# heracles-ec/heracles

Measured on AMD Instinct MI355X. Metric: map->Cl pairs/sec + mixing-matrix build sec, nside=4096 lmax=6144, higher is better.
Workload: dtype f64

## Files before the change

### heracles_amd/csrc/hx_analysis.hip

```cpp
#include <algorithm>
#include <cmath>
#include <cstdlib>
#include <cstring>

#include "hx_sht_common.h"

namespace hx {
using namespace hxfft;

constexpr int HALF_F = 1;
template <int SPIN>
struct LegCfg {
    static constexpr int NW = SPIN == 0 ? 16 : 8;
    static constexpr int NT = SPIN == 0 ? 1 : 2;
    static constexpr int NOP = SPIN == 0 ? 1 : 2;
    static constexpr int NPAR = (SPIN == 2 && HALF_F) ? 1 : 2;
};
int analysis_f_rows(int spin) { return spin == 0 ? LegCfg<0>::NPAR * LegCfg<0>::NOP : LegCfg<2>::NPAR * LegCfg<2>::NOP; }

struct LegParams {
    PlanDev P;
    const LegTask *__restrict__ tasks;
    const double *__restrict__ F;
    double *__restrict__ partial;
    int m0, ms;
    long long row0;
    int ng;
    int ncol;
    int pcol;
    const MTasks *__restrict__ of_m;
    const long long *__restrict__ arow;
    long long arow0;
    int add_all;
};

template <int SPIN>
__global__ __launch_bounds__(256) void k_fourier_combine(PlanDev P, const double2 *__restrict__ Y, int ncomp, int ng,
                                                         int ncol, int m0, int ms, const double *__restrict__ rw,
                                                         const LegTask *__restrict__ tasks, const MTasks *__restrict__ of_m,
                                                         double *__restrict__ F, int tile0)
{
    constexpr int NOP = LegCfg<SPIN>::NOP;
    __shared__ RingAtM ring_at_m[32];
    const int m = m0 + blockIdx.x * ms;
    const int ty = (int)blockIdx.y + tile0;
    const MTasks mt = of_m[m];
    if (mt.count == 0 || ty < tasks[mt.first].rb0) return;
    if (threadIdx.x < 32) ring_at_m[threadIdx.x] = ring_at_m_of(P, ty * 32 + threadIdx.x, m, rw);
    __syncthreads();
    const int rp = ty * 32 + (threadIdx.x >> 3);
    const int slot = threadIdx.x & 7;
    const bool live = rp < P.nrp;
    const RingAtM ram = ring_at_m[threadIdx.x >> 3];
    constexpr int NPAR = LegCfg<SPIN>::NPAR;
    double *row = F + (((long long)blockIdx.x * P.nrp_pad + rp) * NPAR) * NOP * ncol;
    for (int g = 0; g < ng; ++g) {
        if (SPIN == 0) {
            const int c = g * 8 + slot;
            if (g * NCOL + 2 * slot >= ncol) continue;
            double2 s = make_double2(0.0, 0.0), d = s;
            if (live && c < ncomp) {
                double2 fn, fs;
                ring_modes_ns(P, Y, c, rp, m, ram, fn, fs);
                s = cadd(fn, fs);
                d = csub(fn, fs);
            }
            *reinterpret_cast<double2 *>(row + g * NCOL + 2 * slot) = s;
            *reinterpret_cast<double2 *>(row + ncol + g * NCOL + 2 * slot) = d;
        } else {
            const int f = g * 4 + (slot >> 1), op = slot & 1;
            if (g * NCOL + 4 * (slot >> 1) >= ncol) continue;
            double4 o0 = make_double4(0.0, 0.0, 0.0, 0.0), o1 = o0;
            if (live && 2 * f + 1 < ncomp) {
                double2 qn, qs, un, us;
                ring_modes_ns(P, Y, 2 * f, rp, m, ram, qn, qs);
                ring_modes_ns(P, Y, 2 * f + 1, rp, m, ram, un, us);
                const double2 ppn = cscale(cadd(qn, mul_pi(un)), -0.5), pmn = cscale(csub(qn, mul_pi(un)), -0.5);
                const double2 pps = cscale(cadd(qs, mul_pi(us)), -0.5), pms = cscale(csub(qs, mul_pi(us)), -0.5);
                double4 x, y;
                if (op == 0) {
                    x = make_double4(ppn.x, ppn.y, ppn.y, -ppn.x);
                    y = make_double4(pms.x, pms.y, -pms.y, pms.x);
                } else {
                    x = make_double4(pmn.x, pmn.y, -pmn.y, pmn.x);
                    y = make_double4(pps.x, pps.y, pps.y, -pps.x);
                }
                o0 = make_double4(x.x + y.x, x.y + y.y, x.z + y.z, x.w + y.w);
                o1 = make_double4(x.x - y.x, x.y - y.y, x.z - y.z, x.w - y.w);
            }
            const int col = g * NCOL + 4 * (slot >> 1);
            *reinterpret_cast<double4 *>(row + (0 * NOP + op) * ncol + col) = o0;
            if (NPAR == 2) *reinterpret_cast<double4 *>(row + (1 * NOP + op) * ncol + col) = o1;
        }
    }
}

__device__ __host__ inline int tile_swz(int r) { return r & 15; }
__device__ __host__ inline int ringsel(int q, int k) { return (k & 1) * 16 + 2 * q + (k >> 1); }

template <int K>
__device__ inline int opaque(int v)
{
    asm("; opaque %1" : "+v"(v) : "n"(K));
    return v;
}

__device__ unsigned long long g_exec_flops[2];

template <int SPIN>
struct PipeCfg {
    static constexpr int NW = 4;
    static constexpr int RBS = SPIN == 0 ? 2 : 1;
    static constexpr int NCH = SPIN == 0 ? 2 : 1;
    static constexpr int NOP = SPIN == 0 ? 1 : 2;
};

__device__ __host__ inline int pipe_rho(int q, int k) { return 4 * q + k; }
__device__ __host__ inline int pipe_tile_idx(int c, int r) { return c * 32 + ((r ^ (c & 7)) * 2); }

constexpr int DUO_GAP = -1;
constexpr int DUO_PRIO = 1;
constexpr int DUO_ORDER = -1;
constexpr int DUO_SCALE_BITS2 = 100;
constexpr int DUO_SCALE_BITS0 = 300;

template <int K>
__device__ __forceinline__ double row_bcast(double v)
{
    double d;
    asm("v_mov_b64_dpp %0, %1 row_newbcast:%2 row_mask:0xf bank_mask:0xf" : "=v"(d) : "v"(v), "n"(K));
    return d;
}

template <int K>
__device__ __forceinline__ double row_bcast_fmac(double t, double p, double x)
{
    asm("v_fmac_f64_dpp %0, %1, %2 row_newbcast:%3 row_mask:0xf bank_mask:0xf" : "+v"(t) : "v"(p), "v"(x), "n"(K));
    return t;
}

template <int SPIN>
__device__ __forceinline__ void alm_rows_to_layout(const PlanDev &P, int m, bool any_task, const double *__restrict__ partial, long long r0, int ncol,
                                                   int ncomp, int ng, const double *__restrict__ fl, int add, double2 *__restrict__ alm,
                                                   long long alm_stride, const double *__restrict__ alphan, int tid, int nt)
{
    const int lmax = P.lmax;
    const int l0 = SPIN == 0 ? m : (m > 2 ? m : 2);
    const int nl = lmax - m + 1, nc = 8 * ng;
    constexpr int U = 8;
    for (int i0 = tid; i0 < nl * nc; i0 += nt * U) {
        double2 v[U];
        double al[U], f[U];
        long long dsti[U];
        bool on[U];
#pragma unroll
        for (int u = 0; u < U; ++u) {
            const int i = i0 + u * nt;
            const int l = m + i / nc, c = i % nc;
            on[u] = i < nl * nc && c < ncomp;
            v[u] = make_double2(0.0, 0.0);
            al[u] = 1.0;
            f[u] = 1.0;
            dsti[u] = 0;
            if (!on[u]) continue;
            dsti[u] = (long long)c * alm_stride + almidx(lmax, l, m);
            if (l >= l0 && any_task) {
                const double *prow = partial + (r0 + (l - l0)) * ncol + (c >> 3) * NCOL;
                v[u] = *reinterpret_cast<const double2 *>(prow + 2 * (c & 7));
                if (SPIN == 2 && alphan && ((l + m) & 1)) {
                    const int j = 2 * (c & 7);
                    v[u] = make_double2(prow[j ^ 3], prow[(j + 1) ^ 3]);
                }
                if (SPIN == 2 && HALF_F && ((l + m) & 1)) {
                    if (c & 1) v[u].y = -v[u].y;
                    else v[u].x = -v[u].x;
                }
                if (alphan) al[u] = alphan[almidx(lmax, l, m)];
                if (fl) f[u] = fl[l];
            }
        }
#pragma unroll
        for (int u = 0; u < U; ++u) {
            if (!on[u]) continue;
            double2 w = v[u];
            if (alphan) { w.x *= al[u]; w.y *= al[u]; }
            if (fl) { w.x *= f[u]; w.y *= f[u]; }
            double2 *dst = alm + dsti[u];
            if (add) { const double2 o = *dst; w.x += o.x; w.y += o.y; }
            *dst = w;
        }
    }
}

template <int SPIN, int NG, int NBX, int NSUB = 1>
__global__ __launch_bounds__(256, 2) void k_legendre_duo(LegParams A, const double2 *__restrict__ coefn)
{
    using C = PipeCfg<SPIN>;
    constexpr int NW = 4, NOP = C::NOP, NCH = C::NCH, NPAIR = 16;
    constexpr int NXA = NBX > 0 ? NBX : 1;
    constexpr int DQ0 = NG * 512, DSZ = NG * 512 + NBX * 128;
    constexpr bool HALFB = SPIN == 2;
    constexpr int SB = SPIN == 2 ? DUO_SCALE_BITS2 : DUO_SCALE_BITS0;
    constexpr int GAPN = DUO_GAP >= 0 ? DUO_GAP : ((SPIN == 2 && NG == 2 && NBX == 2) ? 5 : (SPIN == 2 && NG == 2 && NBX == 1) ? 6 : (SPIN == 2 && NG == 1 && NBX == 2) ? 0 : 4);
    constexpr int GORDER = DUO_ORDER >= 0 ? DUO_ORDER : ((SPIN == 2 && NG == 2 && NBX == 2) ? 2 : (SPIN == 0 && NG == 1 && NBX == 1) ? 1 : 0);
    constexpr int NPB = HALFB ? 1 : 2;
    constexpr int TW = NSUB * DSZ > 2048 ? NSUB * DSZ : 2048;
    static_assert(NG >= 1 && NG <= 2 && TW * NW * 8 <= 81920, "two work-groups per CU");
    static_assert(SPIN == 0 || HALF_F, "spin 2: the lambda- chain carries (-1)^(l + m) lambda- (one operand row, wave-uniform coefficients)");
    __shared__ double tile[NW][TW];
    __shared__ int lead_in[2][NW];
    const PlanDev &P = A.P;
    const int m = A.m0 + blockIdx.x * A.ms, lmax = P.lmax;
    const MTasks mt = A.of_m[m];
    const int l0 = SPIN == 0 ? m : (m > 2 ? m : 2);
    const int off = (l0 + m) & 1;
    const int nblk = (lmax - l0) / LBLK + 1;
    const long long orow = A.arow[m] - A.arow0;
    const double2 *__restrict__ cfm = coefn + almidx(lmax, 0, m) + l0 + (SPIN == 0 ? 0 : 1) + (threadIdx.x & 15);
    bool first_group = true;
    auto put = [&](double *p, double v) __attribute__((always_inline)) {
        if (first_group) *p = v;
        else __builtin_amdgcn_global_atomic_fadd_f64((__attribute__((address_space(1))) double *)p, v);
    };
    auto lds_barrier = []() __attribute__((always_inline)) {
        __builtin_amdgcn_s_waitcnt(0xc07f);
        __builtin_amdgcn_s_barrier();
    };
    int n_mf = 0, n_rec = 0;
    if (DUO_PRIO) __builtin_amdgcn_s_setprio(3);
    for (int ti = 0; ti < mt.count; ++ti) {
        const LegTask task = A.tasks[mt.first + ti];
        first_group = ti == 0 && !A.add_all;
        int tid = threadIdx.x;
        asm volatile("; ring group" : "+v"(tid));
        const int w = tid >> 6, lane = tid & 63;
        const int ai = lane & 15, ak = lane >> 4;
        if (ti) __syncthreads();

        const int rbi = SPIN == 0 ? 2 * w + (lane >> 5) : w;
        const int rpl = (task.rb0 + rbi) * RBLK + (lane & 31);
        const bool valid = rbi < task.nrb && rpl < P.nrp;
        const double x = valid ? P.z[rpl] : 0.0;
        const double xx = SPIN == 0 ? x * x : ((lane >> 5) ? -x : x);

        double fr[NPAIR][NPB][NG], frx[NPAIR][NPB][NXA];
#pragma unroll
        for (int sp = 0; sp < NPAIR; ++sp) {
            const int op = SPIN == 0 ? 0 : sp & 1, q = SPIN == 0 ? sp : sp >> 1;
            const int rbq = SPIN == 0 ? 2 * w + (q >> 3) : w;
            const bool on = rbq < task.nrb;
            const long long row = (long long)blockIdx.x * P.nrp_pad + (task.rb0 + rbq) * RBLK + pipe_rho(q & 7, ak);
            if (HALFB) {
                const double *f = A.F + (row * NOP + op) * A.ncol;
#pragma unroll
                for (int g = 0; g < NG; ++g) fr[sp][0][g] = on ? f[g * NCOL + ai] : 0.0;
#pragma unroll
                for (int g = 0; g < NXA; ++g) frx[sp][0][g] = (NBX > 0 && on) ? f[NG * NCOL + 4 * g + (lane & 3)] : 0.0;
            } else {
#pragma unroll
                for (int pos = 0; pos < NPB; ++pos) {
                    const double *f = A.F + ((row * 2 + (pos ^ off)) * NOP + op) * A.ncol;
#pragma unroll
                    for (int g = 0; g < NG; ++g) fr[sp][pos][g] = on ? f[g * NCOL + ai] : 0.0;
#pragma unroll
                    for (int g = 0; g < NXA; ++g) frx[sp][pos][g] = (NBX > 0 && on) ? f[NG * NCOL + 4 * g + (lane & 3)] : 0.0;
                }
            }
        }

        double vc[NCH], vp[NCH];
        int sc[NCH];
#pragma unroll
        for (int c = 0; c < NCH; ++c) { vc[c] = 0.0; vp[c] = 0.0; sc[c] = -100; }
        if (valid) {
            if (SPIN == 0) {
                SVal a = spow(P.sth[rpl], m);
                a.v *= P.mfac[m];
                SVal b = a;
                b.v *= sqrt(2.0 * m + 3.0) * P.z[rpl];
                snorm_small(a);
                snorm_small(b);
                vc[0] = a.v; sc[0] = a.e;
                vc[NCH - 1] = b.v; sc[NCH - 1] = b.e;
            } else {
                SVal sp, sm;
                spin2_seeds(m, P.sth[rpl], P.omz[rpl], P.kfac2[m], sp, sm);
                vc[0] = (lane >> 5) ? (off ? -sm.v : sm.v) : sp.v;
                sc[0] = (lane >> 5) ? sm.e : sp.e;
            }
#pragma unroll
            for (int c = 0; c < NCH; ++c) sval_rebase<SB>(vc[c], sc[c]);
        }

        auto rec_step = [&](auto RMM, int c, int step, const double tq) __attribute__((always_inline)) {
            constexpr int RM = decltype(RMM)::value;
            if (RM != 3 && (step & 3) == 0) {
                const int hc = __double2hiint(vc[c]), hp = __double2hiint(vp[c]);
                const bool up = sc[c] < 0 && (hc & 0x7ff00000) >= 0x3ff00000;
                const int sub = up ? (SB << 20) : 0;
                const bool pz = up && (hp & 0x7ff00000) <= (SB << 20);
                vc[c] = __hiloint2double(hc - sub, __double2loint(vc[c]));
                vp[c] = pz ? 0.0 : __hiloint2double(hp - sub, __double2loint(vp[c]));
                sc[c] += up ? 1 : 0;
            }
            const double cur = (RM == 3 || sc[c] == 0) ? vc[c] : 0.0;
            const double vn = fma(tq, vc[c], -vp[c]);
            vp[c] = vc[c];
            vc[c] = vn;
            return cur;
        };
        constexpr int HB = 8;
        double *tw = &tile[w][0];
        auto recursion = [&](auto RMM, const double2 (&cl)[2]) __attribute__((always_inline)) {
            constexpr int RM = decltype(RMM)::value;
#pragma unroll
            for (int h = 0; h < LBLK / HB; ++h) {
                double cur[HB];
#pragma unroll
                for (int k = 0; k < HB; ++k) {
                    constexpr int dummy = 0; (void)dummy;
                    const int kk = HB * h + k;
                    double tq = 0.0;
                    switch (kk & 15) {
#define HX_BC(K) case K: tq = row_bcast_fmac<K>(row_bcast<K>(cl[kk >> 4].y), cl[kk >> 4].x, xx); break;
                        HX_BC(0) HX_BC(1) HX_BC(2) HX_BC(3) HX_BC(4) HX_BC(5) HX_BC(6) HX_BC(7)
                        HX_BC(8) HX_BC(9) HX_BC(10) HX_BC(11) HX_BC(12) HX_BC(13) HX_BC(14) HX_BC(15)
#undef HX_BC
                    }
                    cur[k] = rec_step(RMM, SPIN == 0 ? ((kk & 1) ? NCH - 1 : 0) : 0, SPIN == 0 ? kk >> 1 : kk, tq);
                }
                if (RM >= 2) {
#pragma unroll
                    for (int j = 0; j < HB / 2; ++j)
                        *reinterpret_cast<double2 *>(tw + pipe_tile_idx(lane, h * (HB / 2) + j)) = make_double2(cur[2 * j], cur[2 * j + 1]);
                }
                __builtin_amdgcn_sched_barrier(0);
            }
        };
        auto set_mode = [&](int b) __attribute__((always_inline)) {
            const int eb = b == 0 ? 60 : (b == 1 ? 34 : (30 - 2 * b > 8 ? 30 - 2 * b : 8));
            auto lane_dead = [&](int c) __attribute__((always_inline)) {
                if (SB == 300) return sc[c] < 0;
                const int ef = (__double2hiint(vc[c]) >> 20) & 0x7ff;
                return sc[c] <= -2 || (sc[c] == -1 && ef <= 1022 - eb);
            };
            bool dead = !valid || lane_dead(0), live = !valid || sc[0] == 0;
            if (NCH == 2) {
                dead = dead && (!valid || lane_dead(NCH - 1));
                live = live && (!valid || sc[NCH - 1] == 0);
            }
            return __all(dead) ? 1 : (__all(live) ? 3 : 2);
        };
        using I1 = std::integral_constant<int, 1>;
        using I2 = std::integral_constant<int, 2>;
        using I3 = std::integral_constant<int, 3>;

        const int fcol = tid & 15, fch = (tid >> 4) & 7, fpos = (tid >> 7) & 1;
        const int frow = (fch >> 1) + 8 * (fch & 1);
        const int qrow = tid / (4 * NXA), qcol = tid % (4 * NXA);
        double *pgrp = A.partial + (orow + 2 * frow + fpos) * A.pcol + fcol;
        double *pquad = A.partial + (orow + 2 * qrow) * A.pcol + NG * NCOL + qcol;
        double2 cnext[2] = {cfm[0], cfm[16]};
        bool started = first_group;
        int nflush = 0;
        for (int b0 = 0; b0 < nblk; b0 += NSUB) {
            double4_t acc[NSUB][NG][2];
            double accx[NSUB][NXA][2];
            bool mine = false;
#pragma unroll
            for (int sub = 0; sub < NSUB; ++sub) {
                const int b = b0 + sub;
#pragma unroll
                for (int g = 0; g < NG; ++g) acc[sub][g][0] = acc[sub][g][1] = (double4_t){0.0, 0.0, 0.0, 0.0};
#pragma unroll
                for (int g = 0; g < NXA; ++g) accx[sub][g][0] = accx[sub][g][1] = 0.0;
                if (b >= nblk) break;
                int rm = set_mode(b);
                const double2 cl[2] = {cnext[0], cnext[1]};
                if (rm == 3) recursion(I3{}, cl);
                else if (rm == 2) {
                    recursion(I2{}, cl);
                    if (SB != 300) {
                        bool lv = valid && sc[0] == 0;
                        if (NCH == 2) lv = lv || (valid && sc[NCH - 1] == 0);
                        if (!__any(lv)) rm = 1;
                    }
                } else recursion(I1{}, cl);
                cnext[0] = cfm[(b + 1) * LBLK];
                cnext[1] = cfm[(b + 1) * LBLK + 16];
                n_rec = __builtin_amdgcn_readfirstlane(n_rec + 1);
                mine = mine || rm >= 2;
                if (rm >= 2) {
                    n_mf = __builtin_amdgcn_readfirstlane(n_mf + 1);
                    if (DUO_PRIO) __builtin_amdgcn_s_setprio(0);
                    constexpr int PF = 3;
                    auto a_fetch = [&](int sp) __attribute__((always_inline)) {
                        const int op = SPIN == 0 ? 0 : sp & 1, q = SPIN == 0 ? sp : sp >> 1;
                        const int c = SPIN == 0 ? (q >> 3) * 32 + pipe_rho(q & 7, ak) : op * 32 + pipe_rho(q, ak);
                        return *reinterpret_cast<const double2 *>(tw + pipe_tile_idx(c, ai));
                    };
                    double2 aq[PF + 1];
#pragma unroll
                    for (int j = 0; j < PF; ++j) aq[j] = a_fetch(j);
#pragma unroll
                    for (int sp = 0; sp < NPAIR; ++sp) {
                        if (sp + PF < NPAIR) aq[(sp + PF) % (PF + 1)] = a_fetch(sp + PF);
                        const double a0 = aq[sp % (PF + 1)].x, a1 = aq[sp % (PF + 1)].y;
#pragma unroll
                        for (int pos = 0; pos < 2; ++pos) {
                            const double a = pos ? a1 : a0;
                            if (GAPN > 0) {
                                if (GORDER == 1) {
#pragma unroll
                                for (int g = 0; g < (NG > NBX ? NG : NBX); ++g) {
                                    if (g < NG) acc[sub][g][pos] = __builtin_amdgcn_mfma_f64_16x16x4f64(a, fr[sp][HALFB ? 0 : pos][g], acc[sub][g][pos], 0, 0, 0);
                                    __builtin_amdgcn_sched_barrier(0);
                                    asm volatile("s_nop %0" ::"n"(GAPN > 0 ? GAPN - 1 : 0));
                                    __builtin_amdgcn_sched_barrier(0);
                                    if (g < NBX) accx[sub][g][pos] = __builtin_amdgcn_mfma_f64_4x4x4f64(a, frx[sp][HALFB ? 0 : pos][g], accx[sub][g][pos], 0, 0, 0);
                                    __builtin_amdgcn_sched_barrier(0);
                                }
                                } else if (GORDER == 2) {
#pragma unroll
                                for (int g = 0; g < NG; ++g) acc[sub][g][pos] = __builtin_amdgcn_mfma_f64_16x16x4f64(a, fr[sp][HALFB ? 0 : pos][g], acc[sub][g][pos], 0, 0, 0);
                                __builtin_amdgcn_sched_barrier(0);
                                asm volatile("s_nop %0" ::"n"(GAPN > 0 ? GAPN - 1 : 0));
                                __builtin_amdgcn_sched_barrier(0);
#pragma unroll
                                for (int g = 0; g < NBX; ++g) accx[sub][g][pos] = __builtin_amdgcn_mfma_f64_4x4x4f64(a, frx[sp][HALFB ? 0 : pos][g], accx[sub][g][pos], 0, 0, 0);
                                __builtin_amdgcn_sched_barrier(0);
                                if (NBX > 0) asm volatile("s_nop %0" ::"n"(GAPN > 0 ? GAPN - 1 : 0));
                                __builtin_amdgcn_sched_barrier(0);
                                } else {
#pragma unroll
                                for (int g = 0; g < (NG > NBX ? NG : NBX); ++g) {
                                    if (g < NG) acc[sub][g][pos] = __builtin_amdgcn_mfma_f64_16x16x4f64(a, fr[sp][HALFB ? 0 : pos][g], acc[sub][g][pos], 0, 0, 0);
                                    if (g < NBX) accx[sub][g][pos] = __builtin_amdgcn_mfma_f64_4x4x4f64(a, frx[sp][HALFB ? 0 : pos][g], accx[sub][g][pos], 0, 0, 0);
                                    __builtin_amdgcn_sched_barrier(0);
                                    asm volatile("s_nop %0" ::"n"(GAPN > 0 ? GAPN - 1 : 0));
                                    __builtin_amdgcn_sched_barrier(0);
                                }
                                }
                            } else {
#pragma unroll
                                for (int g = 0; g < NG; ++g) acc[sub][g][pos] = __builtin_amdgcn_mfma_f64_16x16x4f64(a, fr[sp][HALFB ? 0 : pos][g], acc[sub][g][pos], 0, 0, 0);
#pragma unroll
                                for (int g = 0; g < NBX; ++g) accx[sub][g][pos] = __builtin_amdgcn_mfma_f64_4x4x4f64(a, frx[sp][HALFB ? 0 : pos][g], accx[sub][g][pos], 0, 0, 0);
                            }
                        }
                        __builtin_amdgcn_sched_barrier(0);
                    }
                    if (DUO_PRIO) __builtin_amdgcn_s_setprio(3);
                }
            }
            const bool two = NSUB > 1 && b0 + 1 < nblk;
            if (!started) {
                if (lane == 0) lead_in[nflush & 1][w] = mine ? 1 : 0;
                lds_barrier();
                const int4 fl = *reinterpret_cast<const int4 *>(&lead_in[nflush & 1][0]);
                ++nflush;
                started = __builtin_amdgcn_readfirstlane(fl.x | fl.y | fl.z | fl.w) != 0;
                if (!started) {
                    pgrp += (long long)NSUB * LBLK * A.pcol;
                    pquad += (long long)NSUB * LBLK * A.pcol;
                    continue;
                }
            }
#pragma unroll
            for (int sub = 0; sub < NSUB; ++sub) {
                double *dt = tw + sub * DSZ;
#pragma unroll
                for (int g = 0; g < NG; ++g)
#pragma unroll
                    for (int pos = 0; pos < 2; ++pos)
#pragma unroll
                        for (int h = 0; h < 2; ++h)
                            *reinterpret_cast<double2 *>(dt + (g * 2 + pos) * 256 + ai * 16 + (((2 * ak + h) ^ (ai & 7)) * 2)) = make_double2(acc[sub][g][pos][2 * h], acc[sub][g][pos][2 * h + 1]);
#pragma unroll
                for (int g = 0; g < NBX; ++g)
                    *reinterpret_cast<double2 *>(dt + DQ0 + ((4 * ((lane >> 2) & 3) + ak) * 4 * NBX + 4 * g + (lane & 3)) * 2) = make_double2(accx[sub][g][0], accx[sub][g][1]);
            }
            lds_barrier();
#pragma unroll
            for (int sub = 0; sub < NSUB; ++sub) {
                if (sub > 0 && !two) break;
                const long long rsub = (long long)sub * LBLK * A.pcol;
#pragma unroll
                for (int g = 0; g < NG; ++g) {
                    const double *src = &tile[0][0] + sub * DSZ + (g * 2 + fpos) * 256 + fcol * 16 + ((fch ^ (fcol & 7)) * 2);
                    double2 s4[NW];
#pragma unroll
                    for (int ww = 0; ww < NW; ++ww) s4[ww] = *reinterpret_cast<const double2 *>(src + ww * TW);
                    put(pgrp + rsub + g * NCOL, (s4[0].x + s4[1].x) + (s4[2].x + s4[3].x));
                    put(pgrp + rsub + g * NCOL + 8 * (long long)A.pcol, (s4[0].y + s4[1].y) + (s4[2].y + s4[3].y));
                }
                if (NBX > 0 && tid < 64 * NBX) {
                    double2 s4[NW];
#pragma unroll
                    for (int ww = 0; ww < NW; ++ww) s4[ww] = *reinterpret_cast<const double2 *>(&tile[0][0] + ww * TW + sub * DSZ + DQ0 + tid * 2);
                    put(pquad + rsub, (s4[0].x + s4[1].x) + (s4[2].x + s4[3].x));
                    put(pquad + rsub + A.pcol, (s4[0].y + s4[1].y) + (s4[2].y + s4[3].y));
                }
            }
            pgrp += (long long)NSUB * LBLK * A.pcol;
            pquad += (long long)NSUB * LBLK * A.pcol;
            lds_barrier();
        }
    }
    if ((threadIdx.x & 63) == 0) {
        atomicAdd(&g_exec_flops[0], (unsigned long long)n_mf * (32ull * (NG * 2048ull + NBX * 512ull)));
        atomicAdd(&g_exec_flops[1], (unsigned long long)n_rec * (64ull * LBLK * 4ull));
    }
}

template <int SPIN>
__global__ __launch_bounds__(256) void k_alm_reduce(PlanDev P, const LegTask *__restrict__ tasks,
                                                    const MTasks *__restrict__ of_m,
                                                    const double *__restrict__ partial, long long row0, int m0, int ms,
                                                    int ncomp, int ng, int ncol, const double *__restrict__ fl, int add,
                                                    double2 *__restrict__ alm, long long alm_stride,
                                                    const long long *__restrict__ arow, const double *__restrict__ alphan)
{
    const int m = m0 + blockIdx.x * ms, lmax = P.lmax;
    const int l0 = SPIN == 0 ? m : (m > 2 ? m : 2);
    const MTasks mt = of_m[m];
    const int nl = lmax - m + 1, nc = 8 * ng;
    if (arow) {
        alm_rows_to_layout<SPIN>(P, m, mt.count > 0, partial, arow[m] - row0, ncol, ncomp, ng, fl, add, alm, alm_stride, alphan, threadIdx.x, blockDim.x);
        return;
    }
    for (int i = threadIdx.x; i < nl * nc; i += blockDim.x) {
        const int l = m + i / nc, c = i % nc;
        if (c >= ncomp) continue;
        double2 v = make_double2(0.0, 0.0);
        if (l >= l0) {
            const int col = (c >> 3) * NCOL + 2 * (c & 7);
            for (int t = 0; t < mt.count; ++t) {
                const double *p = partial + (tasks[mt.first + t].pout - row0 + (l - l0)) * ncol + col;
                v.x += p[0];
                v.y += p[1];
            }
            if (fl) { v.x *= fl[l]; v.y *= fl[l]; }
        }
        double2 *dst = alm + (long long)c * alm_stride + almidx(lmax, l, m);
        if (add) { const double2 o = *dst; v.x += o.x; v.y += o.y; }
        *dst = v;
    }
}

__global__ __launch_bounds__(256) void k_alm_reduce_spin(int lmax, int s, const LegTask *__restrict__ tasks, const MTasks *__restrict__ of_m,
                                                         const double *__restrict__ partial, long long row0, int m0, int ms,
                                                         const double *__restrict__ fl, int add, double2 *__restrict__ alm, long long alm_stride)
{
    const int m = m0 + blockIdx.x * ms;
    const int l0 = m > s ? m : s;
    const MTasks mt = of_m[m];
    const int nl = lmax - m + 1;
    for (int i = threadIdx.x; i < nl * 2; i += blockDim.x) {
        const int l = m + (i >> 1), c = i & 1;
        double2 v = make_double2(0.0, 0.0);
        if (l >= l0) {
            for (int t = 0; t < mt.count; ++t) {
                const double *p = partial + (tasks[mt.first + t].pout - row0 + (l - l0)) * 4 + 2 * c;
                v.x += p[0];
                v.y += p[1];
            }
            if (fl) { v.x *= fl[l]; v.y *= fl[l]; }
        }
        double2 *dst = alm + (long long)c * alm_stride + almidx(lmax, l, m);
        if (add) { const double2 o = *dst; v.x += o.x; v.y += o.y; }
        *dst = v;
    }
}

struct SweepShape {
    int ng, nbx, valu, ncol, duo;
};
static SweepShape sweep_shape(int spin, int nb)
{
    const int cols = 2 * nb;
    SweepShape sh = {0, 0, 0, 0, 0};
    if (cols <= 8) { sh.valu = 1; return sh; }
    sh.duo = 1;
    sh.ng = std::max(cols / NCOL, 1);
    const int rem = cols > NCOL ? cols % NCOL : 0;
    const int maxbx = spin == 2 ? 2 : (sh.ng == 1 ? 1 : 0);
    if (rem > 4 * maxbx) sh.ng += 1;
    else sh.nbx = (rem + 3) / 4;
    sh.ncol = NCOL * sh.ng + 4 * sh.nbx;
    return sh;
}
bool analysis_generic_spin(int spin)
{
    if (spin != 2) return spin != 0;
    const char *e = getenv("HX_SPIN_GENERIC");
    return e && atoi(e) != 0;
}
int analysis_max_comp(int spin) { return spin == 2 ? 8 * NGMAX + 4 : 8 * NGMAX; }

static double sweep_cost(int spin, int units)
{
    if (spin == 0) return units <= 4 ? 21.6 * units : (units <= 8 ? 84.1 : (units <= 10 ? 99.2 : 139.7));
    return units <= 2 ? 61.0 * units : (units <= 4 ? 164.5 : (units == 5 ? 194.1 : (units == 6 ? 222.0 : (units <= 8 ? 272.0 : (units == 9 ? 299.6 : 326.0)))));
}
int analysis_next_batch(int spin, int remaining)
{
    const int unit = spin == 0 ? 1 : 2, maxu = analysis_max_comp(spin) / unit;
    const int units = remaining / unit;
    if (units <= 0) return 0;
    std::vector<double> best(units + 1, 0.0);
    std::vector<int> first(units + 1, 0);
    for (int r = 1; r <= units; ++r) {
        best[r] = 1e300;
        for (int b = std::min(maxu, r); b >= 1; --b) {
            const double c = sweep_cost(spin, b) + best[r - b];
            if (c < best[r] - 1e-9) { best[r] = c; first[r] = b; }
        }
    }
    return unit * first[units];
}
int analysis_max_batch(int spin, int ncomp)
{
    int mx = 0;
    for (int left = ncomp; left > 0;) {
        const int nb = analysis_next_batch(spin, left);
        if (nb <= 0) break;
        mx = std::max(mx, nb);
        left -= nb;
    }
    return mx;
}

int one_set_task_blocks(int spin) { return PipeCfg<2>::NW * (spin ? PipeCfg<2>::RBS : PipeCfg<0>::RBS); }
int flop_task_blocks(int spin) { return spin == 0 ? LegCfg<0>::NW : LegCfg<2>::NW; }

static bool duo_shape(const SweepShape &sh) { return sh.duo != 0; }
static int sweep_pcol(const SweepShape &sh) { return sh.ncol > 2 * NCOL ? (sh.ncol + 15) / 16 * 16 : sh.ncol; }

template <int SPIN>
static int launch_duo(const SweepShape &sh, dim3 pgrid, hipStream_t st, const LegParams &A, const double2 *cn)
{
    const dim3 db(256);
    const int key = sh.ng * 10 + sh.nbx;
    if (key == 10) hipLaunchKernelGGL((k_legendre_duo<SPIN, 1, 0, 2>), pgrid, db, 0, st, A, cn);
    else if (key == 11) hipLaunchKernelGGL((k_legendre_duo<SPIN, 1, 1, 2>), pgrid, db, 0, st, A, cn);
    else if (key == 20 && SPIN == 2) hipLaunchKernelGGL((k_legendre_duo<2, 2, 0, 2>), pgrid, db, 0, st, A, cn);
    else if (key == 12 && SPIN == 2) hipLaunchKernelGGL((k_legendre_duo<2, 1, 2, 2>), pgrid, db, 0, st, A, cn);
    else if (key == 21 && SPIN == 2) hipLaunchKernelGGL((k_legendre_duo<2, 2, 1, 2>), pgrid, db, 0, st, A, cn);
    else if (key == 20) hipLaunchKernelGGL((k_legendre_duo<SPIN, 2, 0>), pgrid, db, 0, st, A, cn);
    else if (key == 22 && SPIN == 2) hipLaunchKernelGGL((k_legendre_duo<2, 2, 2>), pgrid, db, 0, st, A, cn);
    else return fail(HX_ERR_ARG, "legendre analysis: no two-group kernel for %d groups + %d blocks", sh.ng, sh.nbx);
    return HX_OK;
}

static void launch_alm_reduce(hx_plan *pl, int spin, hx_plan::TaskSet &ts, long long row0, int m0, int ms, int nm, int nb, int ng, int pcol,
                              const double *d_fl, int add, double2 *d_alms, const double *al)
{
    const PlanDev P = pl->dev();
    const long long *arow = al ? ts.d_arow.as<long long>() : nullptr;
    if (spin == 0)
        hipLaunchKernelGGL(k_alm_reduce<0>, dim3(nm), dim3(256), 0, rt().stream, P, ts.d_tasks.as<LegTask>(), ts.d_of_m.as<MTasks>(), pl->partial.as<double>(),
                           row0, m0, ms, nb, ng, pcol, d_fl, add, d_alms, pl->nlm, arow, al);
    else
        hipLaunchKernelGGL(k_alm_reduce<2>, dim3(nm), dim3(256), 0, rt().stream, P, ts.d_tasks.as<LegTask>(), ts.d_of_m.as<MTasks>(), pl->partial.as<double>(),
                           row0, m0, ms, nb, ng, pcol, d_fl, add, d_alms, pl->nlm, arow, al);
}

template <int SPIN>
static int launch_chunk(hx_plan *pl, hx_plan::SpinData &sd, hx_plan::TaskSet &ts, int m0, int m1, int nb, const SweepShape &sh, const double *d_rw,
                        const double *d_fl, int add, double2 *d_alms)
{
    const int ng = sh.ng + (sh.nbx > 0 ? 1 : 0), ncol = sh.ncol;
    const int pcol = sweep_pcol(sh);
    hipStream_t st = rt().stream;
    PlanDev P = pl->dev();
    const int t0 = ts.of_m[m0].first;
    const int t1 = ts.of_m[m1 - 1].first + ts.of_m[m1 - 1].count;
    const int ms = std::max(pl->m_step, 1), nm = (m1 - m0 + ms - 1) / ms;
    {
        ProfScope ps("fourier_combine");
        dim3 grid(nm, pl->nrp_pad / 32);
        hipLaunchKernelGGL(k_fourier_combine<SPIN>, grid, dim3(256), 0, st, P, pl->Y.as<double2>(), nb, ng, ncol, m0, ms, d_rw,
                           ts.d_tasks.as<LegTask>(), ts.d_of_m.as<MTasks>(), pl->F.as<double>(), 0);
    }
    if (t1 > t0) {
        ProfScope ps("legendre_analysis");
        ProfScope ps2(SPIN == 0 ? "legendre_analysis_s0" : "legendre_analysis_s2");
        LegParams A;
        A.P = P; A.tasks = ts.d_tasks.as<LegTask>() + t0; A.F = pl->F.as<double>(); A.partial = pl->partial.as<double>();
        A.m0 = m0; A.ms = ms; A.row0 = ts.rows_before_m[m0]; A.ng = ng; A.ncol = ncol; A.pcol = pcol;
        A.of_m = ts.d_of_m.as<MTasks>(); A.arow = ts.d_arow.as<long long>(); A.arow0 = ts.arow[m0]; A.add_all = 0;
        A.tasks = ts.d_tasks.as<LegTask>();
        HX_TRY(launch_duo<SPIN>(sh, dim3((unsigned)nm), st, A, sd.cn.as<double2>()));
    }
    {
        ProfScope ps("alm_reduce");
        launch_alm_reduce(pl, SPIN, ts, ts.arow[m0], m0, ms, nm, nb, ng, pcol, d_fl, add, d_alms, sd.al.as<double>());
    }
    HX_HIP(hipGetLastError());
    return HX_OK;
}

static bool valu_batch(int spin, int nb) { return sweep_shape(spin, nb).valu != 0; }

static double analysis_budget(const hx_plan *pl)
{
    if (scratch_budget_bytes() > 0.0) return scratch_budget_bytes();
    double budget = 80e9;
    size_t fr = 0, tot = 0;
    if (hipMemGetInfo(&fr, &tot) == hipSuccess) budget = std::min(budget, 0.5 * (double)(fr + pl->F.bytes + pl->partial.bytes));
    return std::max(budget, 2e9);
}

static int plan_m_chunks(hx_plan *pl, double f_per_m, const std::vector<long long> &prow, size_t row_bytes, std::vector<std::pair<int, int>> &chunks)
{
    const double budget = analysis_budget(pl);
    size_t maxF = 16, maxP = 16;
    const int m_end = pl->m_hi < 0 ? pl->lmax + 1 : std::min(pl->m_hi, pl->lmax + 1), ms = std::max(pl->m_step, 1);
    for (int m0 = std::max(pl->m_lo, 0); m0 < m_end;) {
        int last = m0;
        while (last + ms < m_end) {
            const double bytes = f_per_m * ((last + ms - m0) / ms + 1) + (double)(prow[last + ms + 1] - prow[m0]) * row_bytes;
            if (bytes > budget) break;
            last += ms;
        }
        const int m1 = last + 1;
        chunks.emplace_back(m0, m1);
        maxF = std::max(maxF, (size_t)(f_per_m * ((m1 - m0 + ms - 1) / ms)));
        maxP = std::max(maxP, (size_t)(prow[m1] - prow[m0]) * row_bytes);
        m0 = last + ms;
    }
    HX_TRY(pl->F.alloc(maxF));
    HX_TRY(pl->partial.alloc(maxP));
    pl->last_chunks = (int)chunks.size();
    return HX_OK;
}

static int analysis_batch_valu(hx_plan *pl, int spin, int nb, const double *d_maps, double2 *d_alms, const double *d_rw,
                               const double *d_pw, const double *d_fl, int add, bool generic = false)
{
    hx_plan::SpinData *sd = nullptr;
    hx_plan::TaskSet *tsp = nullptr;
    HX_TRY(spin_data(pl, spin, generic, &sd));
    HX_TRY(task_set(pl, spin, generic, valu_task_blocks(spin), &tsp));
    hx_plan::TaskSet &ts = *tsp;
    if (pl->hsrc == nullptr && pl->nssrc == nullptr) {
        HX_TRY(pl->Y.alloc(sizeof(double2) * (size_t)pl->ny * nb));
        HX_TRY(launch_ring_subdft_maps(pl, nb, d_maps, d_pw, pl->Y.as<double2>()));
    }
    const int lmax = pl->lmax, pcol = valu_partial_cols(spin), unit = spin ? 2 : 1, ms = std::max(pl->m_step, 1);
    std::vector<std::pair<int, int>> chunks;
    HX_TRY(plan_m_chunks(pl, (double)pl->nrp_pad * valu_operand_doubles(spin) * sizeof(double), ts.rows_before_m, pcol * sizeof(double), chunks));
    for (int c0 = 0; c0 < nb; c0 += unit)
        for (auto &ch : chunks) {
            const int m0 = ch.first, m1 = ch.second, nm = (m1 - m0 + ms - 1) / ms;
            HX_TRY(launch_valu_chunk(pl, spin, *sd, ts, m0, m1, c0, d_rw, generic));
            ProfScope ps("alm_reduce");
            if (generic)
                hipLaunchKernelGGL(k_alm_reduce_spin, dim3(nm), dim3(256), 0, rt().stream, lmax, spin, ts.d_tasks.as<LegTask>(), ts.d_of_m.as<MTasks>(),
                                   pl->partial.as<double>(), ts.rows_before_m[m0], m0, ms, d_fl, add, d_alms + (size_t)c0 * pl->nlm, pl->nlm);
            else
                launch_alm_reduce(pl, spin, ts, ts.rows_before_m[m0], m0, ms, nm, unit, 1, pcol, d_fl, add, d_alms + (size_t)c0 * pl->nlm, nullptr);
            HX_HIP(hipGetLastError());
        }
    return HX_OK;
}

int analysis_batch(hx_plan *pl, int spin, int nb, const double *d_maps, double2 *d_alms, const double *d_rw,
                   const double *d_pw, const double *d_fl, int add)
{
    const bool generic = plan_generic_spin(pl, spin);
    if (generic || (spin != 0 && spin != 2)) {
        if (!generic) return fail(HX_ERR_UNSUPPORTED, "spin-%d maps not yet supported", spin);
        if (spin < 0 || nb < 2 || (nb & 1)) return fail(HX_ERR_ARG, "analysis_batch: %d components of spin %d", nb, spin);
        if (spin > pl->lmax) {
            if (!add) HX_HIP(hipMemsetAsync(d_alms, 0, sizeof(double2) * (size_t)pl->nlm * nb, rt().stream));
            return HX_OK;
        }
        return analysis_batch_valu(pl, spin, nb, d_maps, d_alms, d_rw, d_pw, d_fl, add, true);
    }
    if (valu_batch(spin, nb)) return analysis_batch_valu(pl, spin, nb, d_maps, d_alms, d_rw, d_pw, d_fl, add);
    const SweepShape sh = sweep_shape(spin, nb);
    hx_plan::TaskSet *ts = nullptr;
    hx_plan::SpinData *sd = nullptr;
    HX_TRY(spin_data(pl, spin, false, &sd));
    HX_TRY(task_set(pl, spin, false, one_set_task_blocks(spin), &ts));
    if (pl->hsrc == nullptr && pl->nssrc == nullptr) {
        HX_TRY(pl->Y.alloc(sizeof(double2) * (size_t)pl->ny * nb));
        HX_TRY(launch_ring_subdft_maps(pl, nb, d_maps, d_pw, pl->Y.as<double2>()));
    }
    std::vector<std::pair<int, int>> chunks;
    HX_TRY(plan_m_chunks(pl, (double)pl->nrp_pad * analysis_f_rows(spin) * sh.ncol * sizeof(double), ts->arow, sweep_pcol(sh) * sizeof(double), chunks));
    for (auto &ch : chunks) {
        if (spin == 0)
            HX_TRY(launch_chunk<0>(pl, *sd, *ts, ch.first, ch.second, nb, sh, d_rw, d_fl, add, d_alms));
        else
            HX_TRY(launch_chunk<2>(pl, *sd, *ts, ch.first, ch.second, nb, sh, d_rw, d_fl, add, d_alms));
    }
    return HX_OK;
}

bool analysis_can_stream(hx_plan *pl, int spin, int nb)
{
    if (!pl || pl->nside < 1 || pl->hsrc || pl->nssrc || pl->m_lo != 0 || pl->m_hi >= 0 || pl->m_step > 1) return false;
    if (nb < 1 || nb > analysis_max_comp(spin)) return false;
    const SweepShape sh = sweep_shape(spin, nb);
    if (!duo_shape(sh) || sh.valu) return false;
    const double f_bytes = (double)pl->nrp_pad * analysis_f_rows(spin) * sh.ncol * sizeof(double) * (pl->lmax + 1.0);
    const double p_bytes = 0.5 * (pl->lmax + 1.0) * (pl->lmax + 2.0 + LBLK) * sweep_pcol(sh) * sizeof(double);
    double budget = 80e9;
    if (scratch_budget_bytes() > 0.0) budget = scratch_budget_bytes();
    if (f_bytes + p_bytes > budget) return false;
    size_t fr = 0, tot = 0;
    if (hipMemGetInfo(&fr, &tot) != hipSuccess) {
        (void)hipGetLastError();
        return false;
    }
    const double y_bytes = (double)pl->ny * nb * sizeof(double2), stage_bytes = 2.0 * nb * (double)pl->npix * sizeof(double);
    const double held = (double)pl->F.bytes + (double)pl->partial.bytes + (double)pl->Y.bytes + (double)pl->stage[0].bytes + (double)pl->stage[1].bytes +
                        (double)pl->stage[2].bytes;
    return f_bytes + p_bytes + y_bytes + stage_bytes <= 0.95 * ((double)fr + held);
}

int analysis_stream_plan(hx_plan *pl, int spin, int nb, int nslab, StreamSweep &s)
{
    if (!analysis_can_stream(pl, spin, nb)) return fail(HX_ERR_ARG, "analysis_stream_plan: not a streamable sweep");
    HX_TRY(spin_data(pl, spin, false, &s.sd));
    HX_TRY(task_set(pl, spin, false, one_set_task_blocks(spin), &s.ts));
    hx_plan::TaskSet &ts = *s.ts;
    const SweepShape sh = sweep_shape(spin, nb);
    s.pl = pl; s.spin = spin; s.nb = nb;
    const int nrb = (pl->nrp + RBLK - 1) / RBLK;
    std::vector<double> cum(nrb + 1, 0.0);
    for (int rb = 0; rb < nrb; ++rb) {
        double px = 0.0;
        for (int rp = rb * RBLK; rp < std::min((rb + 1) * RBLK, pl->nrp); ++rp) px += (rp == pl->nrp - 1 ? 4.0 : 8.0) * pl->h_nsub[rp];
        cum[rb + 1] = cum[rb] + px;
    }
    nslab = std::max(1, std::min(nslab, nrb));
    s.rp_edge.assign(1, 0);
    for (int k = 1; k < nslab; ++k) {
        const int rb = (int)(std::lower_bound(cum.begin(), cum.end(), cum[nrb] * k / nslab) - cum.begin());
        if (rb * RBLK > s.rp_edge.back() && rb < nrb) s.rp_edge.push_back(rb * RBLK);
    }
    s.rp_edge.push_back(nrb * RBLK);
    s.nslab = (int)s.rp_edge.size() - 1;
    const int lmax = pl->lmax;
    std::vector<MTasks> tab((size_t)s.nslab * (lmax + 1), MTasks{0, 0});
    for (int m = 0; m <= lmax; ++m) {
        const MTasks mt = ts.of_m[m];
        int t = mt.first;
        for (int k = 0; k < s.nslab; ++k) {
            const int rb_hi = s.rp_edge[k + 1] / RBLK;
            MTasks &o = tab[(size_t)k * (lmax + 1) + m];
            o.first = t;
            while (t < mt.first + mt.count && ts.tasks[t].rb0 + ts.tasks[t].nrb <= rb_hi) ++t;
            o.count = t - o.first;
        }
        if (t != mt.first + mt.count) return fail(HX_ERR_ARG, "analysis_stream_plan: ring groups of m = %d left over", m);
    }
    HX_TRY(upload(s.d_of_m, tab));
    HX_TRY(pl->Y.alloc(sizeof(double2) * (size_t)pl->ny * nb));
    HX_TRY(pl->F.alloc((size_t)pl->nrp_pad * analysis_f_rows(spin) * sh.ncol * sizeof(double) * (size_t)(lmax + 1)));
    HX_TRY(pl->partial.alloc((size_t)ts.arow[lmax + 1] * sweep_pcol(sh) * sizeof(double)));
    return HX_OK;
}

int analysis_stream_start(StreamSweep &s)
{
    hx_plan *pl = s.pl;
    const SweepShape sh = sweep_shape(s.spin, s.nb);
    HX_HIP(hipMemsetAsync(pl->partial.p, 0, (size_t)s.ts->arow[pl->lmax + 1] * sweep_pcol(sh) * sizeof(double), rt().stream));
    pl->last_chunks = 1;
    return HX_OK;
}

template <int SPIN>
static int stream_slab(StreamSweep &s, int k)
{
    hx_plan *pl = s.pl;
    hx_plan::TaskSet &ts = *s.ts;
    const SweepShape sh = sweep_shape(SPIN, s.nb);
    const int ng = sh.ng + (sh.nbx > 0 ? 1 : 0), lmax = pl->lmax, nm = lmax + 1;
    const int rp_lo = s.rp_edge[k], rp_hi = s.rp_edge[k + 1];
    hipStream_t st = rt().stream;
    PlanDev P = pl->dev();
    HX_TRY(launch_ring_subdft_maps(pl, s.nb, s.d_maps, s.d_pw, pl->Y.as<double2>(), rp_lo, std::min(rp_hi, pl->nrp)));
    {
        ProfScope ps("fourier_combine");
        const int tile_hi = k + 1 == s.nslab ? pl->nrp_pad / 32 : rp_hi / 32;
        dim3 grid(nm, tile_hi - rp_lo / 32);
        hipLaunchKernelGGL(k_fourier_combine<SPIN>, grid, dim3(256), 0, st, P, pl->Y.as<double2>(), s.nb, ng, sh.ncol, 0, 1, s.d_rw,
                           ts.d_tasks.as<LegTask>(), ts.d_of_m.as<MTasks>(), pl->F.as<double>(), rp_lo / 32);
    }
    {
        ProfScope ps("legendre_analysis");
        ProfScope ps2(SPIN == 0 ? "legendre_analysis_s0" : "legendre_analysis_s2");
        LegParams A;
        A.P = P; A.tasks = ts.d_tasks.as<LegTask>(); A.F = pl->F.as<double>(); A.partial = pl->partial.as<double>();
        A.m0 = 0; A.ms = 1; A.row0 = 0; A.ng = ng; A.ncol = sh.ncol; A.pcol = sweep_pcol(sh);
        A.of_m = s.d_of_m.as<MTasks>() + (size_t)k * (lmax + 1); A.arow = ts.d_arow.as<long long>(); A.arow0 = 0; A.add_all = 1;
        HX_TRY(launch_duo<SPIN>(sh, dim3((unsigned)nm), st, A, s.sd->cn.as<double2>()));
    }
    HX_HIP(hipGetLastError());
    return HX_OK;
}

int analysis_stream_slab(StreamSweep &s, int k)
{
    if (k < 0 || k >= s.nslab) return fail(HX_ERR_ARG, "analysis_stream_slab: slab %d of %d", k, s.nslab);
    return s.spin == 0 ? stream_slab<0>(s, k) : stream_slab<2>(s, k);
}

int analysis_stream_end(StreamSweep &s)
{
    hx_plan *pl = s.pl;
    const SweepShape sh = sweep_shape(s.spin, s.nb);
    ProfScope ps("alm_reduce");
    launch_alm_reduce(pl, s.spin, *s.ts, 0LL, 0, 1, pl->lmax + 1, s.nb, sh.ng + (sh.nbx > 0 ? 1 : 0), sweep_pcol(sh), s.d_fl, 0, s.d_alms, s.sd->al.as<double>());
    HX_HIP(hipGetLastError());
    return HX_OK;
}

static int flop_wave_blocks(hx_plan *pl, int spin, double *out)
{
    hx_plan::TaskSet *ts = nullptr;
    HX_TRY(task_set(pl, spin, false, flop_task_blocks(spin), &ts));
    *out = 0.0;
    for (const LegTask &t : ts->tasks) *out += (double)t.nrb * ((pl->lmax - std::max(t.m, spin)) / LBLK + 1);
    return HX_OK;
}

}

extern "C" int hx_plan_mfma_flops(hx_plan *pl, int spin, int ncomp, double *flops)
{
    using namespace hx;
    if (!pl || !flops || ncomp < 1 || (spin != 0 && spin != 2)) return fail(HX_ERR_ARG, "hx_plan_mfma_flops: bad arguments");
    HX_TRY(ensure_ready());
    double wave_blocks = 0.0;
    HX_TRY(flop_wave_blocks(pl, spin, &wave_blocks));
    const int nop = spin ? 2 : 1;
    double per_wave_block = 0.0;
    for (int c0 = 0, nb = 0; c0 < ncomp; c0 += nb) {
        nb = analysis_next_batch(spin, ncomp - c0);
        const SweepShape sh = sweep_shape(spin, nb);
        per_wave_block += 16.0 * nop * (sh.ng * 2048.0 + sh.nbx * 512.0);
    }
    *flops = wave_blocks * per_wave_block;
    return HX_OK;
}

extern "C" int hx_executed_flops(double *out2, int reset)
{
    using namespace hx;
    if (!out2) return fail(HX_ERR_ARG, "hx_executed_flops: null output");
    HX_TRY(ensure_ready());
    HX_HIP(hipStreamSynchronize(rt().stream));
    unsigned long long v[2] = {0, 0}, w = 0;
    HX_HIP(hipMemcpyFromSymbol(v, HIP_SYMBOL(g_exec_flops), sizeof(v)));
    HX_TRY(valu_exec_flops(&w, reset != 0));
    if (reset) {
        const unsigned long long z[2] = {0, 0};
        HX_HIP(hipMemcpyToSymbol(HIP_SYMBOL(g_exec_flops), z, sizeof(z)));
    }
    out2[0] = (double)v[0];
    out2[1] = (double)v[1] + (double)w;
    return HX_OK;
}

extern "C" int hx_plan_executed_flops(hx_plan *pl, int spin, int ncomp, double *out2)
{
    using namespace hx;
    if (!out2) return fail(HX_ERR_ARG, "hx_plan_executed_flops: null output");
    HX_TRY(hx_plan_mfma_flops(pl, spin, ncomp, &out2[0]));
    double wave_blocks = 0.0;
    HX_TRY(flop_wave_blocks(pl, spin, &wave_blocks));
    const int nop = spin ? 2 : 1;
    int sweeps = 0;
    for (int c0 = 0, nb = 0; c0 < ncomp; c0 += nb, ++sweeps) nb = analysis_next_batch(spin, ncomp - c0);
    out2[1] = wave_blocks * sweeps * (double)RBLK * LBLK * nop * 4.0;
    return HX_OK;
}
```

Baseline: 424.0.

## Tile fourier_combine over m×ring blocks staged in LDS with XCD-aware block swizzle

Restructures the Fourier-combine kernel so each block handles a tile of 16 m values times 4 or 8 ring pairs. Results are assembled in dynamic LDS and then written to F as contiguous coalesced double2 rows per m. Blocks are remapped across 8 XCDs so neighbouring tiles share an L2. Thread count and ring-pair count adapt to row length, with up to 1024 threads. This targets scattered Y reads and poorly coalesced F writes, at the cost of more LDS use, extra synchronisation, and more complex indexing.

```diff
diff --git a/heracles_amd/csrc/hx_analysis.hip b/heracles_amd/csrc/hx_analysis.hip
--- a/heracles_amd/csrc/hx_analysis.hip
+++ b/heracles_amd/csrc/hx_analysis.hip
@@ -34,42 +34,69 @@
     int add_all;
 };
 
-template <int SPIN>
-__global__ __launch_bounds__(256) void k_fourier_combine(PlanDev P, const double2 *__restrict__ Y, int ncomp, int ng,
-                                                         int ncol, int m0, int ms, const double *__restrict__ rw,
+constexpr int COMB_NXCD = 8, COMB_XG = 4;
+constexpr int COMB_TM = 16;
+constexpr int COMB_IPT = 3;
+constexpr int COMB_MPAD = 2;
+static int combine_rp(int rowlen) { return rowlen <= 40 ? 8 : 4; }
+static size_t combine_lds_bytes(int rp, int rowlen)
+{
+    return (size_t)COMB_TM * ((size_t)rp * rowlen + COMB_MPAD) * sizeof(double) + (size_t)COMB_TM * rp * sizeof(RingAtM) + COMB_TM * sizeof(int);
+}
+template <int SPIN, int RP>
+__global__ __launch_bounds__(1024) void k_fourier_combine(PlanDev P, const double2 *__restrict__ Y, int ncomp, int ncol, int m0, int ms,
+                                                         int nm, int kshift, int gx, int gy, const double *__restrict__ rw,
                                                          const LegTask *__restrict__ tasks, const MTasks *__restrict__ of_m,
                                                          double *__restrict__ F, int tile0)
 {
-    constexpr int NOP = LegCfg<SPIN>::NOP;
-    __shared__ RingAtM ring_at_m[32];
-    const int m = m0 + blockIdx.x * ms;
-    const int ty = (int)blockIdx.y + tile0;
-    const MTasks mt = of_m[m];
-    if (mt.count == 0 || ty < tasks[mt.first].rb0) return;
-    if (threadIdx.x < 32) ring_at_m[threadIdx.x] = ring_at_m_of(P, ty * 32 + threadIdx.x, m, rw);
+    constexpr int NOP = LegCfg<SPIN>::NOP, NPAR = LegCfg<SPIN>::NPAR, TM = COMB_TM;
+    const int bq = (int)blockIdx.x / (COMB_NXCD * COMB_XG), br = (int)blockIdx.x % (COMB_NXCD * COMB_XG);
+    const int t = (bq * COMB_NXCD + br % COMB_NXCD) * COMB_XG + br / COMB_NXCD;
+    if (t >= gx * gy) return;
+    const int tx = t % gx, ty = t / gx;
+    static_assert(TM == 16 && 32 % RP == 0 && TM * RP <= 256, "tile shape");
+    extern __shared__ __align__(16) unsigned char comb_lds[];
+    const int rowlen = NPAR * NOP * ncol;
+    const int mstride = RP * rowlen + COMB_MPAD;
+    double *tile = reinterpret_cast<double *>(comb_lds);
+    RingAtM *ring_at_m = reinterpret_cast<RingAtM *>(tile + TM * mstride);
+    int *m_live = reinterpret_cast<int *>(ring_at_m + TM * RP);
+    const int kb = tx * TM - kshift;
+    const int rp0 = (ty + tile0 * (32 / RP)) * RP;
+    if (threadIdx.x < TM * RP) {
+        const int mi = threadIdx.x % TM, j = threadIdx.x / TM, k = kb + mi;
+        bool on = k >= 0 && k < nm;
+        if (on) {
+            const int m = m0 + k * ms;
+            const MTasks mt = of_m[m];
+            on = mt.count != 0 && rp0 / 32 >= tasks[mt.first].rb0;
+            if (on) ring_at_m[j * TM + mi] = ring_at_m_of(P, rp0 + j, m, rw);
+        }
+        if (j == 0) m_live[mi] = on;
+    }
     __syncthreads();
-    const int rp = ty * 32 + (threadIdx.x >> 3);
-    const int slot = threadIdx.x & 7;
-    const bool live = rp < P.nrp;
-    const RingAtM ram = ring_at_m[threadIdx.x >> 3];
-    constexpr int NPAR = LegCfg<SPIN>::NPAR;
-    double *row = F + (((long long)blockIdx.x * P.nrp_pad + rp) * NPAR) * NOP * ncol;
-    for (int g = 0; g < ng; ++g) {
+    const int nsl = ncol >> 1;
+    for (int e = threadIdx.x; e < RP * nsl * TM; e += blockDim.x) {
+        const int i = e % TM, sj = e / TM, s = sj % nsl, j = sj / nsl;
+        const int mi = ((i & 3) << 2) | (i >> 2);
+        if (!m_live[mi]) continue;
+        const int m = m0 + (kb + mi) * ms, rp = rp0 + j;
+        const bool live = rp < P.nrp;
+        const RingAtM ram = ring_at_m[j * TM + mi];
+        double *row = tile + mi * mstride + j * rowlen;
         if (SPIN == 0) {
-            const int c = g * 8 + slot;
-            if (g * NCOL + 2 * slot >= ncol) continue;
-            double2 s = make_double2(0.0, 0.0), d = s;
+            const int c = s;
+            double2 sm = make_double2(0.0, 0.0), d = sm;
             if (live && c < ncomp) {
                 double2 fn, fs;
                 ring_modes_ns(P, Y, c, rp, m, ram, fn, fs);
-                s = cadd(fn, fs);
+                sm = cadd(fn, fs);
                 d = csub(fn, fs);
             }
-            *reinterpret_cast<double2 *>(row + g * NCOL + 2 * slot) = s;
-            *reinterpret_cast<double2 *>(row + ncol + g * NCOL + 2 * slot) = d;
+            *reinterpret_cast<double2 *>(row + 2 * s) = sm;
+            *reinterpret_cast<double2 *>(row + ncol + 2 * s) = d;
         } else {
-            const int f = g * 4 + (slot >> 1), op = slot & 1;
-            if (g * NCOL + 4 * (slot >> 1) >= ncol) continue;
+            const int f = s >> 1, op = s & 1;
             double4 o0 = make_double4(0.0, 0.0, 0.0, 0.0), o1 = o0;
             if (live && 2 * f + 1 < ncomp) {
                 double2 qn, qs, un, us;
@@ -88,11 +115,45 @@
                 o0 = make_double4(x.x + y.x, x.y + y.y, x.z + y.z, x.w + y.w);
                 o1 = make_double4(x.x - y.x, x.y - y.y, x.z - y.z, x.w - y.w);
             }
-            const int col = g * NCOL + 4 * (slot >> 1);
-            *reinterpret_cast<double4 *>(row + (0 * NOP + op) * ncol + col) = o0;
-            if (NPAR == 2) *reinterpret_cast<double4 *>(row + (1 * NOP + op) * ncol + col) = o1;
-        }
-    }
+            double2 *t0 = reinterpret_cast<double2 *>(row + (0 * NOP + op) * ncol + 4 * f);
+            t0[0] = make_double2(o0.x, o0.y);
+            t0[1] = make_double2(o0.z, o0.w);
+            if (NPAR == 2) {
+                double2 *t1 = reinterpret_cast<double2 *>(row + (1 * NOP + op) * ncol + 4 * f);
+                t1[0] = make_double2(o1.x, o1.y);
+                t1[1] = make_double2(o1.z, o1.w);
+            }
+        }
+    }
+    __syncthreads();
+    const int lane = threadIdx.x & 63, npiece = RP * rowlen / 2, cpm = (npiece + 63) / 64;
+    for (int ch = threadIdx.x >> 6; ch < TM * cpm; ch += blockDim.x >> 6) {
+        const int mi = ch / cpm, u = (ch % cpm) * 64 + lane;
+        if (!m_live[mi] || u >= npiece) continue;
+        const double2 *src = reinterpret_cast<const double2 *>(tile + mi * mstride);
+        double2 *dst = reinterpret_cast<double2 *>(F + ((long long)(kb + mi) * P.nrp_pad + rp0) * rowlen);
+        dst[u] = src[u];
+    }
+}
+
+template <int SPIN>
+static void launch_fourier_combine(hipStream_t st, const PlanDev &P, const double2 *Y, int ncomp, int ncol, int m0, int ms, int nm, const double *d_rw,
+                                   const LegTask *tasks, const MTasks *of_m, double *F, int tile0, int ntile32)
+{
+    const int kshift = ms == 1 ? m0 % COMB_TM : 0;
+    const int rowlen = LegCfg<SPIN>::NPAR * LegCfg<SPIN>::NOP * ncol;
+    const int gx = (nm + kshift + COMB_TM - 1) / COMB_TM;
+    static_assert((size_t)COMB_TM * (4 * LegCfg<SPIN>::NPAR * LegCfg<SPIN>::NOP * (NCOL * NGMAX + 8) + COMB_MPAD) * sizeof(double) +
+                          (size_t)COMB_TM * 4 * sizeof(RingAtM) + COMB_TM * sizeof(int) <= 65536, "a tile of 4 ring pairs must fit 64 KiB of LDS");
+    const int rp = combine_rp(rowlen), items = rp * (ncol / 2) * COMB_TM;
+    const unsigned nt = (unsigned)std::min(1024, std::max(COMB_TM * rp, (items / COMB_IPT + 63) / 64 * 64));
+    const int gy = ntile32 * (32 / rp);
+    const dim3 grid((unsigned)((gx * gy + COMB_NXCD * COMB_XG - 1) / (COMB_NXCD * COMB_XG) * (COMB_NXCD * COMB_XG)));
+    const size_t lds = combine_lds_bytes(rp, rowlen);
+    if (rp == 8)
+        hipLaunchKernelGGL((k_fourier_combine<SPIN, 8>), grid, dim3(nt), lds, st, P, Y, ncomp, ncol, m0, ms, nm, kshift, gx, gy, d_rw, tasks, of_m, F, tile0);
+    else
+        hipLaunchKernelGGL((k_fourier_combine<SPIN, 4>), grid, dim3(nt), lds, st, P, Y, ncomp, ncol, m0, ms, nm, kshift, gx, gy, d_rw, tasks, of_m, F, tile0);
 }
 
 __device__ __host__ inline int tile_swz(int r) { return r & 15; }
@@ -679,9 +740,8 @@
     const int ms = std::max(pl->m_step, 1), nm = (m1 - m0 + ms - 1) / ms;
     {
         ProfScope ps("fourier_combine");
-        dim3 grid(nm, pl->nrp_pad / 32);
-        hipLaunchKernelGGL(k_fourier_combine<SPIN>, grid, dim3(256), 0, st, P, pl->Y.as<double2>(), nb, ng, ncol, m0, ms, d_rw,
-                           ts.d_tasks.as<LegTask>(), ts.d_of_m.as<MTasks>(), pl->F.as<double>(), 0);
+        launch_fourier_combine<SPIN>(st, P, pl->Y.as<double2>(), nb, ncol, m0, ms, nm, d_rw, ts.d_tasks.as<LegTask>(), ts.d_of_m.as<MTasks>(),
+                                     pl->F.as<double>(), 0, pl->nrp_pad / 32);
     }
     if (t1 > t0) {
         ProfScope ps("legendre_analysis");
@@ -889,9 +949,8 @@
     {
         ProfScope ps("fourier_combine");
         const int tile_hi = k + 1 == s.nslab ? pl->nrp_pad / 32 : rp_hi / 32;
-        dim3 grid(nm, tile_hi - rp_lo / 32);
-        hipLaunchKernelGGL(k_fourier_combine<SPIN>, grid, dim3(256), 0, st, P, pl->Y.as<double2>(), s.nb, ng, sh.ncol, 0, 1, s.d_rw,
-                           ts.d_tasks.as<LegTask>(), ts.d_of_m.as<MTasks>(), pl->F.as<double>(), rp_lo / 32);
+        launch_fourier_combine<SPIN>(st, P, pl->Y.as<double2>(), s.nb, sh.ncol, 0, 1, nm, s.d_rw, ts.d_tasks.as<LegTask>(), ts.d_of_m.as<MTasks>(),
+                                     pl->F.as<double>(), rp_lo / 32, tile_hi - rp_lo / 32);
     }
     {
         ProfScope ps("legendre_analysis");
```

Measured after the change: 430.2 (median of 6 runs). 1.01x the previous value.
